# msi-se/generalized-icp

Hardware: AMD Instinct MI355X
Metric: GICP iterations/sec (and ms/iter) at N points, 1/2/4/8 GPU; final transform error (higher is better)
Workload: dtype f32-screen+f64; 1 GPU; 3d_room_1000k_1000k_k20; n_target=1000000, dim=3, k=20, parallelism=dp1 (one GPU, no collective)

## Files before the change

### generalized-icp_amd/csrc/gicp_kernels.hip

```cpp
#include <hip/hip_runtime.h>

#include <algorithm>
#include <utility>

#include "gicp_internal.h"
#include "gicp_solver.h"
#include "gicp_solve_dev.h"

namespace gicp {

__device__ __forceinline__ int lane_id() { return __lane_id(); }
__device__ __forceinline__ unsigned umed3(unsigned a, unsigned b, unsigned c) {
    return max(min(a, b), min(max(a, b), c));
}
__device__ __forceinline__ float key_d2(unsigned k) { return __uint_as_float(k & ~63u); }
__device__ __forceinline__ float marg(const Margin& m, float d2) {
    return fmaf(m.a * 1.0001f, __builtin_amdgcn_sqrtf(d2), fmaf(m.c, d2, m.b));
}

#define GICP_WAVE_REDUCE(OP, ID, x)                                                      \
    x = OP(x, __builtin_amdgcn_update_dpp(ID, x, 0x111, 0xf, 0xf, false));               \
    x = OP(x, __builtin_amdgcn_update_dpp(ID, x, 0x112, 0xf, 0xf, false));               \
    x = OP(x, __builtin_amdgcn_update_dpp(ID, x, 0x114, 0xf, 0xf, false));               \
    x = OP(x, __builtin_amdgcn_update_dpp(ID, x, 0x118, 0xf, 0xf, false));               \
// ... 312 lines not shown
        qa.ew[a] = 0.5f * (hi - lo) + 4.8e-7f * (fabsf(lo) + fabsf(hi) + B) + 1e-30f;
    }
    return qa;
}

struct NoCount {
    __device__ __forceinline__ void count(int, unsigned = 1) {}
};
template <int D, class Visit, class WB, class Collect, class Cnt = NoCount>
__device__ __forceinline__ void traverse_c(const DevCloud& db, const Query<D>& q, int seed, Visit&& visit,
                                           WB&& wave_bound, float skin, Collect&& collect, Cnt* cnt = nullptr) {
    const int l = lane_id();
    auto infl = [&](float w) -> float {
        if (skin <= 0.f || w < 0.f) return w;
        const float r = __builtin_amdgcn_sqrtf(w) * 1.0001f + skin;
        return r * r;
    };
    float wb = wave_bound();
    float wbi = infl(wb);
    if (seed >= 0) {
        collect(seed);
        if (visit(seed)) {
            wb = wave_bound();
            wbi = infl(wb);
        }
    }
    typedef __attribute__((address_space(4))) const BlockInfo* ConstBlocks;
    const ConstBlocks cb0 = (ConstBlocks)(uintptr_t)db.blocks + db.nblocks;
    for (int b0 = 0; b0 < db.nblocks; b0 += kWave) {
        {
            const ConstBlocks sb = cb0 + (b0 / kWave);
            const double c[3] = {sb->c[0], sb->c[1], sb->c[2]};
            const float h[3] = {sb->h[0], sb->h[1], sb->h[2]};
            if (!__builtin_amdgcn_readfirstlane((int)(gap2_box<D>(q, c, h) <= wbi))) continue;
        }
        if (cnt) cnt->count(5);
        const int b = b0 + l;
        bool cb = false;
        if (b < db.nblocks) cb = gap2_box<D>(q, db.blocks[b].c, db.blocks[b].h) <= wbi;
        uint64_t bm = __ballot(cb);
        while (bm) {
            const int bb = b0 + __ffsll((unsigned long long)bm) - 1;
            bm &= bm - 1;
            const int first = db.blocks[bb].first, nt = db.blocks[bb].ntiles;
            if (cnt) cnt->count(6);
            const int t = first + l;
            bool ct = false, cv = false;
            if (l < nt && t != seed) {
                const float g2 = gap2_box<D>(q, db.tiles[t].c, db.tiles[t].h);
                ct = g2 <= wbi;
                cv = g2 <= wb;
            }
            if (skin > 0.f) {
                uint64_t cm = __ballot(ct);
                while (cm) {
                    collect(first + __ffsll((unsigned long long)cm) - 1);
                    cm &= cm - 1;
                }
            }
            uint64_t tm = __ballot(cv);
            while (tm) {
                const int T = first + __ffsll((unsigned long long)tm) - 1;
                tm &= tm - 1;
                if (visit(T)) {
                    wb = wave_bound();
                    wbi = infl(wb);
                }
            }
        }
    }
}

template <int D, class Visit, class WB>
__device__ __forceinline__ void traverse(const DevCloud& db, const Query<D>& q, int seed, Visit&& visit,
                                         WB&& wave_bound) {
    traverse_c<D>(db, q, seed, visit, wave_bound, 0.f, [](int) {});
}

struct WaveStage {
    float x[kTile], y[kTile], z[kTile];
    double x64[kTile], y64[kTile], z64[kTile];
    int32_t perm[kTile];
};
constexpr int kStatRow = 17;
constexpr int kStatU = 12, kStatV = 10;
struct WaveStat {
    double u[kStatU * kStatRow];
    double v[kStatV * kStatRow];
};
union __attribute__((aligned(16))) WaveLds {
    WaveStage t;
    WaveStat st;
};

template <int D>
__device__ __forceinline__ float lane_gap2(const Query<D>& q, const TileInfo& ti, float* pr) {
    float g2 = 0.f;
#pragma unroll
    for (int a = 0; a < D; ++a) {
        pr[a] = q.pw[a] + (float)(q.ow[a] - ti.c[a]);
        const float ap = fabsf(pr[a]);
        float g = ap - ti.h[a] - (ap + ti.h[a]) * 9.5367431640625e-7f;
        g = fmaxf(g, 0.f);
        g2 = fmaf(g, g, g2);
    }
    return g2;
}

typedef __attribute__((address_space(4))) const TileInfo* ConstTiles;
__device__ __forceinline__ TileInfo tile_meta(const DevCloud& db, int T) {
    const ConstTiles ct = (ConstTiles)(uintptr_t)db.tiles + __builtin_amdgcn_readfirstlane(T);
    TileInfo t;
#pragma unroll
    for (int a = 0; a < 3; ++a) {
        t.c[a] = ct->c[a];
        t.h[a] = ct->h[a];
    }
    t.start = ct->start;
    t.count = ct->count;
    t.radius = ct->radius;
#pragma unroll
    for (int g = 0; g < kSub; ++g)
#pragma unroll
        for (int a = 0; a < 3; ++a) {
            t.sc[a][g] = ct->sc[a][g];
            t.sh[a][g] = ct->sh[a][g];
        }
    return t;
}

__device__ __forceinline__ void stage_f32(const DevCloud& db, const TileInfo& ti, WaveLds& L) {
    const int l = lane_id();
    float4 v = make_float4(1e30f, 1e30f, 1e30f, 0.f);
    if (l < ti.count) v = db.rel32[ti.start + l];
    L.t.x[l] = v.x;
    L.t.y[l] = v.y;
    L.t.z[l] = v.z;
    wave_sync();
}
__device__ __forceinline__ float4 load_rel(const DevCloud& db, int start, int count) {
    const int l = lane_id();
    float4 v = make_float4(1e30f, 1e30f, 1e30f, 0.f);
    if (l < count) v = db.rel32[start + l];
    return v;
}
__device__ __forceinline__ void stage_f32_from(const float4& v, WaveLds& L) {
    const int l = lane_id();
    L.t.x[l] = v.x;
    L.t.y[l] = v.y;
    L.t.z[l] = v.z;
    wave_sync();
}
template <int D, class VisitPre, class WB, class Collect, class Cnt = NoCount>
__device__ __forceinline__ void walk_c(const DevCloud& db, const Query<D>& q, int seed, VisitPre&& visit_pre,
                                       WB&& wave_bound, float skin, Collect&& collect, Cnt* cnt = nullptr) {
    const int l = lane_id();
    auto infl = [&](float w) -> float {
        if (skin <= 0.f || w < 0.f) return w;
        const float r = __builtin_amdgcn_sqrtf(w) * 1.0001f + skin;
        return r * r;
    };
    float wb = wave_bound();
    float wbi = infl(wb);
    if (seed >= 0) {
        collect(seed);
        if (visit_pre(seed, nullptr)) {
            wb = wave_bound();
// ... 494 lines not shown
            return wave_maxf(amb ? b64 + 2.f * marg(A.mg, b64) : -1.f);
        });
    }

    if (q.valid) {
        A.cov_out[i] = cov_descriptor<D>(S, A.min_nb, A.eps_a, A.m_scale);
        A.count_out[i] = (int)S.n;
    }
}

__global__ void __launch_bounds__(256) k_graph_pack(const float4* __restrict__ nb, const float2* __restrict__ nbh,
                                                    int64_t n, uint4* __restrict__ nbq, uint4* __restrict__ nbx,
                                                    int32_t* __restrict__ nbi) {
    const int64_t i = (int64_t)blockIdx.x * blockDim.x + threadIdx.x;
    if (i >= n) return;
    const float2 h = nbh[i];
    const int cnt = __float_as_int(h.y);
    float m = 0.f;
    for (int k = 0; k < cnt; ++k) {
        const float4 v = nb[i * kGraphK + k];
        m = fmaxf(m, fmaxf(fabsf(v.x), fmaxf(fabsf(v.y), fabsf(v.z))));
    }
    const float s = m > 0.f ? m / 32767.f : 1e-30f;
    const float inv = 1.f / s;
    float key[kGraphK];
    int ord[kGraphK];
    for (int k = 0; k < cnt; ++k) {
        const float4 v = nb[i * kGraphK + k];
        const float kk = fmaf(v.z, v.z, fmaf(v.y, v.y, v.x * v.x));
        const int t = __float_as_int(v.w);
        int pos = k;
        while (pos > 0 && (key[pos - 1] > kk || (key[pos - 1] == kk && __float_as_int(nb[i * kGraphK + ord[pos - 1]].w) > t))) {
            key[pos] = key[pos - 1];
            ord[pos] = ord[pos - 1];
            --pos;
        }
        key[pos] = kk;
        ord[pos] = k;
    }
    uint32_t w[2 + 2 * kGraphK];
    w[0] = __float_as_uint(h.x);
    w[1] = __float_as_uint(s);
    int q[4] = {0, 0, 0, 0};
    for (int k = 0; k < kGraphK; ++k) {
        int idx = -1;
        if (k < cnt) {
            const float4 v = nb[i * kGraphK + ord[k]];
            const float c[3] = {v.x, v.y, v.z};
            for (int a = 0; a < 3; ++a) q[a] = max(-32767, min(32767, __float2int_rn(c[a] * inv)));
            idx = __float_as_int(v.w);
            const int64_t d = (int64_t)idx - i;
            q[3] = d >= -32767 && d <= 32767 ? (int)d : kGraphFar;
        }
        w[2 + 2 * k] = ((uint32_t)q[0] & 0xFFFFu) | ((uint32_t)q[1] << 16);
        w[3 + 2 * k] = ((uint32_t)q[2] & 0xFFFFu) | ((uint32_t)q[3] << 16);
        nbi[i * kGraphK + k] = idx;
    }
    for (int c = 0; c < 8; ++c) nbq[i * 8 + c] = make_uint4(w[4 * c], w[4 * c + 1], w[4 * c + 2], w[4 * c + 3]);
    uint32_t x[12] = {};
    for (int k = 0; k < 2 * (kGraphK - kGraphLineA); ++k) x[k] = w[2 + 2 * kGraphLineA + k];
    for (int c = 0; c < 3; ++c) nbx[i * 3 + c] = make_uint4(x[4 * c], x[4 * c + 1], x[4 * c + 2], x[4 * c + 3]);
}

#ifndef GICP_CORR_ATTR
#if defined(GICP_CORR_WAVES_PER_EU)
#define GICP_CORR_ATTR __attribute__((amdgpu_num_sgpr(GICP_CORR_SGPR), amdgpu_waves_per_eu(GICP_CORR_WAVES_PER_EU, GICP_CORR_WAVES_PER_EU)))
#else
#define GICP_CORR_ATTR __attribute__((amdgpu_num_sgpr(GICP_CORR_SGPR), amdgpu_waves_per_eu(6, 6)))
#endif
#endif
#ifndef GICP_CORR_SGPR
#define GICP_CORR_SGPR 100
#endif

template <int D>
struct StatIdx {
    static constexpr int NS = D * (D + 1) / 2;
    static constexpr int pa(int p) { return D == 3 ? (p < 3 ? 0 : (p < 5 ? 1 : 2)) : (p < 2 ? 0 : 1); }
    static constexpr int pb(int p) {
        return D == 3 ? (p == 0 ? 0 : p == 1 ? 1 : p == 2 ? 2 : p == 3 ? 1 : 2) : (p == 0 ? 0 : 1);
    }
};

template <int D>
__device__ __forceinline__ double stat_value(int k, const double (&W)[D][D], const double (&s)[D],
                                             const double (&wr)[D], double rwr) {
    using SI = StatIdx<D>;
    constexpr int NS = SI::NS;
    if (k < NS * NS) {
        const int p = k / NS, qd = k % NS;
        return W[SI::pa(p)][SI::pb(p)] * (s[SI::pa(qd)] * s[SI::pb(qd)]);
    }
    k -= NS * NS;
    if (k < NS * D) return W[SI::pa(k / D)][SI::pb(k / D)] * s[k % D];
    k -= NS * D;
    if (k < NS) return W[SI::pa(k)][SI::pb(k)];
    k -= NS;
    if (k < D * D) return wr[k / D] * s[k % D];
    k -= D * D;
    if (k < D) return wr[k];
    k -= D;
    if (k == 0) return rwr;
    return 1.0;
}

#ifndef GICP_SPARSE_GROUP
#define GICP_SPARSE_GROUP 4
#endif
constexpr int kSparseGroup = GICP_SPARSE_GROUP;

template <int NV>
__device__ bool peer_exchange(const PeerArgs P, uint64_t seq, double* vals) {
    static_assert(NV <= kPeerSlot, "an exchange slot holds the values");
    __shared__ int s_fail;
    const int R = P.n, me = P.rank, tid = (int)threadIdx.x, nt = (int)blockDim.x;
    const int par = (int)(seq & 1u);
    for (int p = 0; p < R; ++p) {
        double* const dst = P.area[p] + kPeerFlagWords + (size_t)(par * kMaxPeers + me) * kPeerSlot;
        for (int k = tid; k < NV; k += nt) __hip_atomic_store(dst + k, vals[k], __ATOMIC_RELAXED, __HIP_MEMORY_SCOPE_SYSTEM);
    }
    __threadfence_system();
    if (tid == 0) s_fail = 0;
    __syncthreads();
    if (tid < R) {
        uint64_t* f = reinterpret_cast<uint64_t*>(P.area[tid]) + par * kMaxPeers + me;
        __hip_atomic_store(f, seq, __ATOMIC_RELEASE, __HIP_MEMORY_SCOPE_SYSTEM);
        if (tid == 0) *P.ctr = seq;
        const uint64_t* g = reinterpret_cast<const uint64_t*>(P.own) + par * kMaxPeers + tid;
        const uint64_t t0 = (uint64_t)wall_clock64();
        while (__hip_atomic_load(g, __ATOMIC_ACQUIRE, __HIP_MEMORY_SCOPE_SYSTEM) != seq) {
            if ((uint64_t)wall_clock64() - t0 > P.timeout) {
                s_fail = 1;
                break;
            }
            __builtin_amdgcn_s_sleep(1);
        }
    }
    __syncthreads();
    if (s_fail) return false;
    __builtin_amdgcn_fence(__ATOMIC_ACQUIRE, "");
    for (int k = tid; k < NV; k += nt) {
        double s = 0.0;
        for (int p = 0; p < R; ++p)
            s += __hip_atomic_load(P.own + kPeerFlagWords + (size_t)(par * kMaxPeers + p) * kPeerSlot + k,
                                   __ATOMIC_RELAXED, __HIP_MEMORY_SCOPE_SYSTEM);
        vals[k] = s;
    }
    __syncthreads();
    return true;
}

__device__ __forceinline__ double probe_value(int rank, int k, int r) {
    return ldexp((double)((rank + 1) * 1000003 + k * 97 + r * 7919), -7);
}
__global__ void __launch_bounds__(64) k_peer_probe(PeerArgs P, int rounds, double* out) {
    __shared__ double v[kPeerSlot];
    __shared__ uint64_t s_seq;
    __shared__ int s_bad;
    if (threadIdx.x == 0) {
        s_seq = *P.ctr;
        s_bad = 0;
    }
    int done = 0;
    for (int r = 0; r < rounds; ++r) {
        for (int k = threadIdx.x; k < kPeerSlot; k += blockDim.x) v[k] = probe_value(P.rank, k, r);
        __syncthreads();
// ... 52 lines not shown
        const void* p0 = A.state;
        const void* p1 = sc.tiles;
        const void* p2 = A.cert_pass;
        const void* p3 = A.hint;
        asm volatile("" ::"s"(p0), "s"(p1), "s"(p2), "s"(p3));
    }
    const ConstState cs0 = (ConstState)(uintptr_t)A.state;
    const TileInfo st = tile_meta(sc, Tq);
    const int cpass0 = ((ConstI32)(uintptr_t)A.cert_pass)[Tq];
    const int hint0 = ((ConstI32)(uintptr_t)A.hint)[Tq];
    const bool done = cs0->converged && !A.single_pass;
    struct {
        double R[9], t[3];
        float R32[9];
    } P;
#pragma unroll
    for (int a = 0; a < D; ++a) {
#pragma unroll
        for (int b = 0; b < D; ++b) {
            P.R[a * D + b] = cs0->T[a * (D + 1) + b];
            P.R32[a * D + b] = (float)P.R[a * D + b];
        }
        P.t[a] = cs0->T[a * (D + 1) + D];
    }

#ifdef GICP_TAIL
    unsigned long long tl[kTailWords] = {};
    __shared__ unsigned s_walk[8];
    if (threadIdx.x < 8) s_walk[threadIdx.x] = 0;
    __syncthreads();
    if (A.tail && blockIdx.x == 0 && threadIdx.x == 0) A.tail[0] = __builtin_amdgcn_s_memrealtime();
#define GICP_TAIL_MARK(k) do { if (A.tail) tl[k] = __builtin_amdgcn_s_memrealtime(); } while (0)
#else
#define GICP_TAIL_MARK(k) do {} while (0)
#endif
    Stamps S;
    S.start();
#ifdef GICP_TIMELINE
    if (A.stamps && l == 0)
        A.stamps[((int64_t)blockIdx.x * kCorrWaves + w) * 20 + 16] = __builtin_amdgcn_s_memrealtime();
    S.ta = tl_after(P.R[0] + st.c[0], cpass0 + hint0 + st.count);
#endif
    if ((A.use_lists || A.cert_j) && blockIdx.x == 0 && threadIdx.x == 0 && !done) {
        double* ring = A.poses + (A.pass % kPoseRing) * 12;
        for (int a = 0; a < 3; ++a) {
            for (int b = 0; b < 3; ++b) ring[a * 3 + b] = (a < D && b < D) ? P.R[a * D + b] : 0.0;
            ring[9 + a] = a < D ? P.t[a] : 0.0;
        }
    }
    int pairs = 0, list_rebuilds = 0, namb_total = 0, ngproved = 0, nwalked = 0;
    if (T < 0 && done) return;
    if (T >= 0) {
    bool on = false;
    double W[D][D] = {}, sv[D] = {}, wr[D] = {}, rwr = 0.0, r2 = 0.0;
    bool amb = false;
    {
        if (done) return;
        Query<D> q;
        q.valid = l < st.count;
        int i = st.start + min(l, st.count - 1);
        auto refresh_i = [&]() {
            i = st.start + min(lane_id(), st.count - 1);
            asm volatile("" : "+v"(i));
        };
        const float4 rel = sc.rel32[i];
        const float relv[3] = {rel.x, rel.y, rel.z};
#pragma unroll
        for (int a = 0; a < D; ++a) {
            double o = P.t[a];
            float pw = 0.f, ew = 0.f;
#pragma unroll
            for (int b = 0; b < D; ++b) {
                o += P.R[a * D + b] * st.c[b];
                pw = fmaf(P.R32[a * D + b], relv[b], pw);
                ew = fmaf(fabsf(P.R32[a * D + b]), st.h[b], ew);
            }
            q.ow[a] = o;
            q.pw[a] = pw;
            q.ew[a] = ew * (1.0f + 4.8e-7f) + 1e-30f;
        }
        const bool lists = A.use_lists != 0;

        int seed = hint0;
        if (seed < 0 || seed >= tg.ntiles) {
            const uint32_t code = morton_code(q.ow, D, tg.lo, tg.scale, tg.bits);
            int lo = 0, hi = tg.ntiles - 1;
            if (tg.seed_tab) {
                const uint32_t b = code >> tg.seed_shift;
                lo = tg.seed_tab[b];
                hi = tg.seed_tab[b + 1];
            }
            while (lo < hi) {
                const int mid = (lo + hi + 1) >> 1;
                if (tg.tile_code[mid] <= code) lo = mid;
                else hi = mid - 1;
            }
            seed = lo;
        }

        auto disp_since = [&](int bp) -> float {
            if (bp < 0 || A.pass - bp <= 0 || A.pass - bp >= kPoseRing) return -1.f;
            const double* Pb = A.poses + (bp % kPoseRing) * 12;
            double dc2 = 0.0, dr2 = 0.0;
#pragma unroll
            for (int a = 0; a < D; ++a) {
                double m = P.t[a] - Pb[9 + a];
#pragma unroll
                for (int b = 0; b < D; ++b) {
                    const double dr = P.R[a * D + b] - Pb[a * 3 + b];
                    m += dr * st.c[b];
                    dr2 += dr * dr;
                }
                dc2 += m * m;
            }
            return (__builtin_amdgcn_sqrtf((float)dc2) + __builtin_amdgcn_sqrtf((float)dr2) * st.radius) * 1.0001f + 1e-30f;
        };

        bool cert = false;
        int cj = -1;
        float cgap = 0.f, cdelta = -1.f;
        int jp = -1;
        if (A.cert_j) {
            jp = A.cert_j[i];
            const float g0 = A.cert_gap[i];
            cdelta = disp_since(cpass0);
            if constexpr (D == 3) cdelta = __int_as_float(__builtin_amdgcn_readfirstlane(__float_as_int(cdelta)));
            if (cdelta >= 0.f && q.valid) {
                cj = jp;
                cgap = g0;
                cert = cj >= 0 ? 2.f * cdelta < cgap : cgap - cdelta > A.empty_r;
            }
        }
#ifdef GICP_TIMELINE
        S.tb = tl_after(rel.x + cgap, jp);
#endif
        bool have_jp = false;
        float qr[3] = {0.f, 0.f, 0.f}, d2jp = 0.f;
        uint32_t w0[16];
        if (A.cert_j && q.valid && !cert && jp >= 0 && jp < tg.n) {
            const double4 t4 = reinterpret_cast<const double4*>(tg.xyz64)[jp];
            if (tg.nbq) {
                const uint4* row = tg.nbq + (int64_t)jp * 8;
#pragma unroll
                for (int c = 0; c < 4; ++c) {
                    const uint4 v = row[c];
                    w0[4 * c] = v.x;
                    w0[4 * c + 1] = v.y;
                    w0[4 * c + 2] = v.z;
                    w0[4 * c + 3] = v.w;
                }
            }
            const double tv[3] = {t4.x, t4.y, t4.z};
#pragma unroll
            for (int a = 0; a < D; ++a) {
                qr[a] = (float)(q.ow[a] - tv[a]) + q.pw[a];
                d2jp = fmaf(qr[a], qr[a], d2jp);
            }
            have_jp = true;
        }
        bool gcert = false;
        float ggap = 0.f;
#ifdef GICP_TAIL
        int gwhy = 0;
        int gout = 0;
#define GICP_WHY(k) (gwhy = (k))
#define GICP_OUT(k) (gout = (k))
#else
// ... 74 lines not shown
                        coords(k + 1, cb);
                        const f2v ms = {-sc, -sc};
                        const f2v dx = __builtin_elementwise_fma(ms, f2v{ca[0], cb[0]}, f2v{qr[0], qr[0]});
                        const f2v dy = __builtin_elementwise_fma(ms, f2v{ca[1], cb[1]}, f2v{qr[1], qr[1]});
                        const f2v dz = __builtin_elementwise_fma(ms, f2v{ca[2], cb[2]}, f2v{qr[2], qr[2]});
                        const f2v dd = __builtin_elementwise_fma(dx, dx, __builtin_elementwise_fma(dy, dy, dz * dz));
                        upd(dd.x, k);
                        upd(dd.y, k + 1);
                    };
                    auto entries = [&](int k0, int k1) {
#pragma unroll
                        for (int k = k0; k + 1 < k1; k += 2) entry2(k);
                        if ((k1 - k0) & 1) entry(k1 - 1);
                    };
                    auto reach = [&](int k) -> float {
                        float c[3];
                        coords(k, c);
                        const float ox = sc * c[0], oy = sc * c[1], oz = sc * c[2];
                        return __builtin_amdgcn_sqrtf(fmaf(ox, ox, fmaf(oy, oy, oz * oz)));
                    };
                    entries(0, kGraphHalf);
                    const float d0 = __builtin_amdgcn_sqrtf(d0s);
                    const float e = eq + 0.87f * sc + kGraphErr * (d0 + r);
                    float lc = reach(kGraphHalf - 1) - sc - d0 - 2.f * e;
                    bool need = lc <= __builtin_amdgcn_sqrtf(b1) + 2.f * e;
                    if (wave_any(need)) {
                        if (need) {
                            load_half(4);
                            entries(kGraphHalf, kGraphLineA);
                            lc = reach(kGraphLineA - 1) - sc - d0 - 2.f * e;
                            need = lc <= __builtin_amdgcn_sqrtf(b1) + 2.f * e;
                        }
                        if (wave_any(need)) {
                            if (need) {
                                const uint4* rx = tg.nbx + (int64_t)node * 3;
#pragma unroll
                                for (int c = 0; c < 2; ++c) {
                                    const uint4 v = rx[c];
                                    xb[4 * c] = v.x;
                                    xb[4 * c + 1] = v.y;
                                    xb[4 * c + 2] = v.z;
                                    xb[4 * c + 3] = v.w;
                                }
                                const uint2 v2 = *reinterpret_cast<const uint2*>(rx + 2);
                                xb[8] = v2.x;
                                xb[9] = v2.y;
                                entries(kGraphLineA, kGraphK);
                            }
                        }
                    }
                    if (!need) b2 = fminf(b2, lc * lc);
                    auto next_index = [&]() -> int {
                        const int bd = (int)wb >> 16;
                        return bd != kGraphFar ? node + bd : tg.nbi[(int64_t)node * kGraphK + bk];
                    };
                    const float e1 = __builtin_amdgcn_sqrtf(b1), e2 = __builtin_amdgcn_sqrtf(b2);
                    if (e2 - e1 <= 2.f * e) {
                        tie = d0 + e1 + 2.f * e < r;
                        tfar = r - d0 - e;
                        tnode = node;
                        act = false;
                        if (!tie) GICP_WHY(2);
                    } else if (d0 + e1 + 2.f * e < r) {
                        gcert = true;
                        GICP_OUT(h > 0 ? 3 : bk < 0 ? 1 : 2);
                        cj = bk < 0 ? node : next_index();
                        ggap = fminf(e2, r - d0) - e1 - 2.f * e;
                        act = false;
                    } else if (bk < 0) {
                        act = false;
                        GICP_WHY(1);
                    } else {
                        const float c0 = (float)(((int)(wa << 16)) >> 16), c1 = (float)((int)wa >> 16);
                        const float c2 = (float)(((int)(wb << 16)) >> 16);
                        qr[0] = fmaf(-sc, c0, qr[0]);
                        qr[1] = fmaf(-sc, c1, qr[1]);
                        qr[2] = fmaf(-sc, c2, qr[2]);
                        eq = e;
                        node = next_index();
                    }
                }
            }
            if (act) GICP_WHY(3);
            if (wave_any(tie)) {
                if (tie) {
                    double p64[D];
                    {
                        const double4 s4 = reinterpret_cast<const double4*>(A.src.xyz64)[i];
                        const double s4v[3] = {s4.x, s4.y, s4.z};
#pragma unroll
                        for (int a = 0; a < D; ++a) {
                            double p = P.t[a];
#pragma unroll
                            for (int b = 0; b < D; ++b) p += P.R[a * D + b] * s4v[b];
                            p64[a] = p;
                        }
                    }
                    double bd2 = 1e300, sd2 = 1e300;
                    int bj = -1, bo = 0x7fffffff;
                    auto consider = [&](int t) {
                        const double4 t4 = reinterpret_cast<const double4*>(tg.xyz64)[t];
                        const double tv[3] = {t4.x, t4.y, t4.z};
                        const double d2 = dist2_exact<D>(tv, p64);
                        const int og = tg.perm[t];
                        if (d2 < bd2 || (d2 == bd2 && og < bo)) {
                            sd2 = bd2;
                            bd2 = d2;
                            bj = t;
                            bo = og;
                        } else {
                            sd2 = fmin(sd2, d2);
                        }
                    };
                    consider(tnode);
                    const int32_t* ri = tg.nbi + (int64_t)tnode * kGraphK;
                    for (int k = 0; k < kGraphK; ++k) {
                        const int t = ri[k];
                        if (t >= 0) consider(t);
                    }
                    gcert = bj >= 0;
                    if (gcert) GICP_OUT(4);
                    cj = bj;
                    const double g = (fmin(sqrt(sd2), (double)tfar) - sqrt(bd2)) * (1.0 - 1e-6) - 1e-12;
                    ggap = g > 0.0 ? (float)g * (1.0f - 1e-6f) : 0.f;
                }
            }
            if (gcert) {
                cert = true;
                cgap = ggap;
            }
        }
        const bool any_gcert = wave_any(gcert);
        const bool skip_walk = !wave_any(q.valid && !cert);
#ifdef GICP_TAIL
        if (A.tail) {
            const bool wl = q.valid && !cert;
            const uint64_t wm = __ballot(wl);
            const int cd = __popcll(__ballot(have_jp));
            if (l == 0 && cd) atomicAdd(&s_walk[0], (unsigned)cd);
            for (int k = 1; k <= 4; ++k) {
                const int c = __popcll(__ballot(gout == k));
                if (l == 0 && c) atomicAdd(&s_walk[k], (unsigned)c);
            }
            if (l == 0 && wm) {
                atomicAdd(&s_walk[5], (unsigned)__popcll(wm));
                atomicAdd(&s_walk[6], 1u);
            }
            (void)gwhy;
        }
#endif
        ngproved = __popcll(__ballot(gcert));
        nwalked = skip_walk ? 0 : 1;
#ifdef GICP_TIMELINE
        S.tdesc = tl_after(ngproved, (int)skip_walk);
        S.ndesc = (unsigned)__popcll(__ballot(have_jp));
        S.nwalk = (unsigned)__popcll(__ballot(q.valid && !cert));
        S.nwalk_jp = (unsigned)__popcll(__ballot(q.valid && !cert && have_jp));
#endif
        const float kap = cdelta > A.kappa ? 0.f : A.kappa;

        const unsigned init = __float_as_uint(A.search2) | 63u;
        unsigned best = init, sec = init;
        int best_tile = -1;
        auto bound_of = [&](float b) -> float {
            const float w = b + 2.f * marg(A.mg, b);
            const float r = __builtin_amdgcn_sqrtf(b) + kap;
            return fmaxf(w, r * r);
        };
        float cap = 3e38f;
        if (have_jp && !cert && !skip_walk) cap = bound_of(d2jp + 2.f * marg(A.mg, d2jp)) * 1.0001f;
        auto lane_bound = [&]() -> float {
            if (!q.valid || cert) return -1.f;
            return fminf(cap, fminf(key_d2(sec), bound_of(key_d2(best))));
        };
        float lb = lane_bound();
#ifdef GICP_TIMELINE
        S.wb0 = __builtin_amdgcn_sqrtf(fmaxf(wave_maxf(lb), 0.f));
#endif
        auto inflate = [&](float w) -> float {
            if (w < 0.f) return w;
            const float r = __builtin_amdgcn_sqrtf(w) * 1.0001f + 2.f * A.gap_slack;
            return r * r;
        };
        float lbx = inflate(lb);
        int lvis = -1;
        auto visit_pre = [&](int Tt, const float4* pre) -> bool {
            if (wave_any(lvis == Tt)) return false;
            S.mark(1);
            S.count(0);
            const TileInfo ti = tile_meta(tg, Tt);
            float pr[D];
            if (!wave_any(lane_gap2_ns<D>(q, ti, pr) <= lbx)) {
                S.mark(2);
                return false;
            }
            const unsigned sub = sub_mask_ns<D>(ti, pr, lbx);
            if (pre) stage_f32_from(*pre, L);
            else stage_f32(tg, ti, L);
            S.mark(2);
            unsigned tb = 0xFFFFFFFFu, ts = 0xFFFFFFFFu;
            scan_tile<D>(L, ti.count, pr, [&](unsigned key, int) {
                ts = umed3(tb, ts, key);
                tb = min(tb, key);
            }, sub);
            pairs += rows_scanned(sub, ti.count);
            S.count(1);
            S.count(2, __popc(sub));
            if (tb < best) {
                sec = min(best, ts);
                best = tb;
                best_tile = Tt;
            } else {
                sec = min(sec, tb);
            }
            lb = lane_bound();
            lbx = inflate(lb);
            wave_sync();
            S.mark(3);
            return true;
        };
        S.mark(0);
        bool use = false;
        float delta = 0.f, rc = 0.f;
        int nl = 0;
        if (lists && !skip_walk) {
            nl = A.list_len[T];
            rc = A.list_rcert[T];
            if (nl > 0 && rc > 0.f) {
                delta = disp_since(A.list_pass[T]);
                use = delta >= 0.f && delta < rc;
            }
        }
        int ent = 0;

        const uint64_t walkers = skip_walk ? 0ull : __ballot(lb >= 0.f);
        const bool sparse = walkers != 0ull && __popcll(walkers) <= A.sparse_max;
        auto sparse_search = [&](int wl) {
            float pw[D];
#pragma unroll
            for (int a = 0; a < D; ++a) pw[a] = readlane_f(q.pw[a], wl);
            Query<D> qp = q;
#pragma unroll
            for (int a = 0; a < D; ++a) {
                const float B = 2.f * q.ew[a] + 1e-30f;
                qp.ow[a] = q.ow[a] + (double)pw[a];
                qp.ew[a] = 4.8e-7f * (2.f * fabsf(pw[a]) + B) + 1e-30f;
            }
            const float capw = readlane_f(cap, wl);
            float wb = readlane_f(lb, wl);
            unsigned tb = init, ts = init;
            int tt = -1;
            unsigned wbest = init, wsec = init;
            int wtile = -1;
            const unsigned M = key_mask();
            auto reduce = [&]() {
                wbest = wave_min_key(tb);
                const int win = __ffsll((unsigned long long)__ballot(tb == wbest)) - 1;
                wsec = wave_min_key(l == win ? ts : tb);
                wtile = __builtin_amdgcn_readlane(tt, win);
                wb = fminf(capw, fminf(key_d2(wsec), bound_of(key_d2(wbest))));
            };
            auto screen = [&](uint64_t cm, int ct, int cst, int ccnt, const float* co, float cg) {
                cm &= __ballot(cg <= wb);
                while (cm) {
                    int ks[kSparseGroup];
                    float rx[kSparseGroup], ry[kSparseGroup], rz[kSparseGroup];
#pragma unroll
// ... 170 lines not shown
            };
            walk_c<D>(tg, q, seed, visit_pre, [&]() { return wave_maxf(lb); }, lists ? skin : 0.f,
                      collect, &S);
            if (lists) {
                const float wbf = wave_maxf(lb);
                const float r = ncol <= kListMax ? __builtin_amdgcn_sqrtf(fmaxf(wbf, 0.f)) * 0.9999f + skin : 0.f;
                if (ncol <= kListMax) {
                    float key = 3e38f;
                    if (l < ncol) {
                        key = 0.f;
#pragma unroll
                        for (int a = 0; a < D; ++a) {
                            const float d = (float)(tg.boxes[cent].c[a] - q.ow[a]);
                            key = fmaf(d, d, key);
                        }
                    }
                    wave_sort64(key, cent);
                    if (l < ncol) A.list[(int64_t)T * kListMax + l] = cent;
                }
                if (l == 0) {
                    A.list_len[T] = min(ncol, kListMax);
                    A.list_rcert[T] = r;
                    A.list_pass[T] = A.pass;
                }
            }
        }
        S.mark(1);
#ifdef GICP_TIMELINE
        S.twalk = tl_after(best, best_tile);
        S.kind = skip_walk ? 0u : use_sparse ? 4u : use ? 1u : list_rebuilds > 0 ? 2u : 3u;
#endif

        auto source_point = [&](const double4& s4) {
            const double s4v[3] = {s4.x, s4.y, s4.z};
#pragma unroll
            for (int a = 0; a < D; ++a) {
                double p = P.t[a];
#pragma unroll
                for (int b = 0; b < D; ++b) p += P.R[a * D + b] * s4v[b];
                q.p64[a] = p;
            }
        };
        refresh_i();
        if (!skip_walk) source_point(reinterpret_cast<const double4*>(sc.xyz64)[i]);
        const bool found = cert ? cj >= 0 : (q.valid && best < init);
        int j = -1;
        double d2e = 0.0;
        if (cert) {
            j = cj;
        } else if (found) {
            const float b = key_d2(best), s2 = key_d2(sec);
            amb = (s2 - b) <= marg(A.mg, b) + marg(A.mg, s2);
            j = tg.boxes[best_tile].start + (int)(best & 63u);
        }
        if (A.cert_j && (!skip_walk || any_gcert || A.pass - cpass0 >= kPoseRing / 2)) {
            if (q.valid) {
                float g = 0.f;
                if (gcert) {
                    g = cgap;
                } else if (cert) {
                    g = cj >= 0 ? cgap - 2.f * cdelta : cgap - cdelta;
                } else if (found) {
                    if (!amb) {
                        const float b = key_d2(best), s2 = key_d2(sec);
                        const float lo2 = fminf(s2 - marg(A.mg, s2), lane_bound());
                        const float hi2 = b + marg(A.mg, b);
                        g = (__builtin_amdgcn_sqrtf(fmaxf(lo2, 0.f)) - __builtin_amdgcn_sqrtf(hi2)) * 0.999f;
                    }
                } else {
                    g = __builtin_amdgcn_sqrtf(A.search2 - marg(A.mg, A.search2)) * 0.9999f;
                }
                A.cert_j[i] = cert ? cj : (found && !amb ? j : -1);
                A.cert_gap[i] = (found && amb) ? 0.f : g;
            }
            if (l == 0) A.cert_pass[T] = A.pass;
        }
        const uint64_t fm = __ballot(found && !cert);
        if (fm && A.hint) {
            const int src_lane = __ffsll((unsigned long long)fm) - 1;
            const int bt = __shfl(best_tile, src_lane);
            if (l == 0) A.hint[T] = bt;
        }

        if (!skip_walk && __any(amb)) {
            double bd2 = 1e300;
            float sd2 = 3e38f;
            int bj = -1;
            const float lim = key_d2(best) + 2.f * marg(A.mg, key_d2(best));
            auto visit64 = [&](int Tt) -> bool {
                const TileInfo ti = tile_meta(tg, Tt);
                float pr[D];
                const bool need = amb && lane_gap2<D>(q, ti, pr) <= lim;
                if (!__any(need)) return false;
                S.count(7);
                const unsigned sub = sub_mask<D>(ti, pr, amb, lim);
                stage_f64(tg, ti, L);
                if (l < ti.count) L.t.perm[l] = tg.perm[ti.start + l];
                wave_sync();
                for (int g = 0; g < kSub; ++g) {
                    if (!((sub >> g) & 1u)) continue;
                    const int je = min(kSubRows * g + kSubRows, ti.count);
#pragma unroll 4
                    for (int jj = kSubRows * g; jj < je; ++jj) {
                        const double qq[3] = {L.t.x64[jj], L.t.y64[jj], L.t.z64[jj]};
                        const double d2 = dist2_exact<D>(qq, q.p64);
                        const int og = L.t.perm[jj];
                        if (amb) {
                            if (d2 < bd2 || (d2 == bd2 && bj >= 0 && og < tg.perm[bj])) {
                                sd2 = (float)bd2 * 0.99999976f;
                                bd2 = d2;
                                bj = ti.start + jj;
                            } else {
                                sd2 = fminf(sd2, (float)d2 * 0.99999976f);
                            }
                        }
                    }
                }
                wave_sync();
                return true;
            };
            const uint64_t am = __ballot(amb);
            if (__popcll(am) <= A.sparse_amb) {
                uint64_t wm = am;
                while (wm) {
                    const int wl = __ffsll((unsigned long long)wm) - 1;
                    wm &= wm - 1;
                    double pa[3] = {0.0, 0.0, 0.0};
                    Query<D> qp = q;
#pragma unroll
                    for (int a = 0; a < D; ++a) {
                        pa[a] = readlane_d(q.p64[a], wl);
                        const float pw = readlane_f(q.pw[a], wl);
                        const float B = 2.f * q.ew[a] + 1e-30f;
                        qp.ow[a] = q.ow[a] + (double)pw;
                        qp.ew[a] = 4.8e-7f * (2.f * fabsf(pw) + B) + 1e-30f;
                    }
                    const float limw = readlane_f(lim, wl);
                    double ub = 1e300;
                    int uo = 0x7fffffff, uj = -1;
                    float us = 3e38f;
                    auto screen64 = [&](uint64_t cm, int ts, int tc) {
                        while (cm) {
                            const int k = __ffsll((unsigned long long)cm) - 1;
                            cm &= cm - 1;
                            const int s0 = __builtin_amdgcn_readlane(ts, k), c0 = __builtin_amdgcn_readlane(tc, k);
                            S.count(7);
                            double d2 = 1e300;
                            int og = 0x7fffffff;
                            if (l < c0) {
                                const double4 x = reinterpret_cast<const double4*>(tg.xyz64)[s0 + l];
                                og = tg.perm[s0 + l];
                                const double xv[3] = {x.x, x.y, x.z};
                                d2 = dist2_exact<D>(xv, pa);
                            }
                            const double m = wave_mind(d2);
                            const uint64_t eq = __ballot(d2 == m);
                            const int om = (int)wave_min_key(d2 == m ? (unsigned)og : 0x7fffffffu);
                            const int wn = __ffsll((unsigned long long)__ballot(d2 == m && og == om)) - 1;
                            const double st = __popcll(eq) >= 2 ? m : wave_mind(l == wn ? 1e300 : d2);
                            if (m < ub || (m == ub && om < uo)) {
                                us = fminf(us, fminf((float)ub * 0.99999976f, (float)st * 0.99999976f));
                                ub = m;
                                uo = om;
                                uj = s0 + wn;
                            } else {
                                us = fminf(us, (float)m * 0.99999976f);
                            }
                        }
                    };
                    const int nsuper = (tg.nblocks + kWave - 1) / kWave;
                    for (int s0 = 0; s0 < nsuper; s0 += kWave) {
                        float sg = 3e38f;
                        if (s0 + l < nsuper) sg = gap2_box<D>(qp, tg.blocks[tg.nblocks + s0 + l].c, tg.blocks[tg.nblocks + s0 + l].h);
                        uint64_t sm = __ballot(sg <= limw);
                        while (sm) {
                            const int sl = __ffsll((unsigned long long)sm) - 1;
                            sm &= sm - 1;
                            const int b0 = (s0 + sl) * kWave, b = b0 + l;
                            float bg = 3e38f;
                            if (b < tg.nblocks) bg = gap2_box<D>(qp, tg.blocks[b].c, tg.blocks[b].h);
                            uint64_t bm = __ballot(bg <= limw);
                            while (bm) {
                                const int bl = __ffsll((unsigned long long)bm) - 1;
                                bm &= bm - 1;
                                const int first = (b0 + bl) * kBlockTiles, nt = min(kBlockTiles, tg.ntiles - first);
// ... 91 lines not shown
                    W[0][1] = W[1][0] = -S[0][1] * id;
                } else {
                    const double c00 = S[1][1] * S[2][2] - S[1][2] * S[2][1];
                    const double c01 = S[0][2] * S[2][1] - S[0][1] * S[2][2];
                    const double c02 = S[0][1] * S[1][2] - S[0][2] * S[1][1];
                    const double c11 = S[0][0] * S[2][2] - S[0][2] * S[2][0];
                    const double c12 = S[0][2] * S[1][0] - S[0][0] * S[1][2];
                    const double c22 = S[0][0] * S[1][1] - S[0][1] * S[1][0];
                    const double det = S[0][0] * c00 + S[0][1] * c01 + S[0][2] * c02;
                    const double id = solver_detail::recip(det);
                    W[0][0] = c00 * id;
                    W[0][1] = W[1][0] = c01 * id;
                    W[0][2] = W[2][0] = c02 * id;
                    W[1][1] = c11 * id;
                    W[1][2] = W[2][1] = c12 * id;
                    W[2][2] = c22 * id;
                }
                }
                double r[D];
#pragma unroll
                for (int a = 0; a < D; ++a) r[a] = qv[a] - q.p64[a];
                r2 = 0.0;
#pragma unroll
                for (int a = 0; a < D; ++a) r2 += r[a] * r[a];
                rwr = 0.0;
#pragma unroll
                for (int a = 0; a < D; ++a) {
                    wr[a] = 0.0;
#pragma unroll
                    for (int b = 0; b < D; ++b) wr[a] += W[a][b] * r[b];
                    rwr += r[a] * wr[a];
                }
            }
            if (A.dbg_index) A.dbg_index[sc.perm[i]] = on ? (int64_t)tg.perm[j] : -1;
        } else if (q.valid) {
            if (skip_walk) source_point(s4e);
            if (A.dbg_index) A.dbg_index[sc.perm[i]] = -1;
            if (A.dbg_dist) A.dbg_dist[sc.perm[i]] = 1.0 / 0.0;
        }
        if (A.dbg_det && q.valid) {
            double dt = 0.0;
            if (on) {
                if constexpr (D == 2) dt = W[0][0] * W[1][1] - W[0][1] * W[1][0];
                else
                    dt = W[0][0] * (W[1][1] * W[2][2] - W[1][2] * W[2][1]) -
                         W[0][1] * (W[1][0] * W[2][2] - W[1][2] * W[2][0]) +
                         W[0][2] * (W[1][0] * W[2][1] - W[1][1] * W[2][0]);
            }
            A.dbg_det[i] = dt;
            A.top_tgt[i] = on ? (int64_t)tg.perm[j] : -1;
        }
        if (A.dbg_weight && q.valid) {
            double* o = A.dbg_weight + (int64_t)sc.perm[i] * D * D;
#pragma unroll
            for (int a = 0; a < D; ++a)
#pragma unroll
                for (int b = 0; b < D; ++b) o[a * D + b] = on ? W[a][b] : 0.0;
        }
        amb = amb && q.valid;
    }

    S.mark(5);
    {
        constexpr int NS = D * (D + 1) / 2;
        constexpr int NU = NS + D + 3;
        constexpr int NV = NS + D + 1;
        auto uel = [&](int k) -> double {
            if (k < NS) return W[StatIdx<D>::pa(k)][StatIdx<D>::pb(k)];
            if (k < NS + D) return wr[k - NS];
            if (k == NS + D) return rwr;
            if (k == NS + D + 1) return on ? 1.0 : 0.0;
            return r2;
        };
        auto vel = [&](int k) -> double {
            if (k < NS) return sv[StatIdx<D>::pa(k)] * sv[StatIdx<D>::pb(k)];
            if (k < NS + D) return sv[k - NS];
            return 1.0;
        };
        typedef double d4v __attribute__((ext_vector_type(4)));
        d4v acc = {0.0, 0.0, 0.0, 0.0};
        WaveStat& X = s_lds[w].st;
        static_assert(NU <= kStatU && NV <= kStatV, "statistics terms fit the transpose image");
        const uint64_t onm = __ballot(on);
        wave_sync();
        double* const wu = &X.u[l & 15];
        double* const wv = &X.v[l & 15];
        const double* const ru = &X.u[min(l & 15, NU - 1) * kStatRow + (l >> 4)];
        const double* const rv = &X.v[min(l & 15, NV - 1) * kStatRow + (l >> 4)];
#pragma unroll
        for (int g = 0; g < 4; ++g) {
            if (((onm >> (16 * g)) & 0xFFFFull) == 0) continue;
            if ((l >> 4) == g) {
#pragma unroll
                for (int k = 0; k < NU; ++k) wu[k * kStatRow] = uel(k);
#pragma unroll
                for (int k = 0; k < NV; ++k) wv[k * kStatRow] = vel(k);
            }
            wave_sync();
#pragma unroll
            for (int cc = 0; cc < 4; ++cc) {
                if (((onm >> (16 * g + 4 * cc)) & 0xFull) == 0) continue;
                acc = __builtin_amdgcn_mfma_f64_16x16x4f64(ru[4 * cc], rv[4 * cc], acc, 0, 0, 0);
            }
            wave_sync();
        }
        double* const wst = wstat(w);
        for (int k = l; k < NSX; k += 64) wst[k] = 0.0;
#pragma unroll
        for (int j = 0; j < 4; ++j) {
            const int p = (l >> 4) + 4 * j, qq = l & 15;
            int idx = -1;
            if (p < NS) {
                if (qq < NS) idx = p * NS + qq;
                else if (qq < NS + D) idx = NS * NS + p * D + (qq - NS);
                else if (qq == NS + D) idx = NS * NS + NS * D + p;
            } else if (p < NS + D) {
                if (qq >= NS && qq < NS + D) idx = NS * NS + NS * D + NS + (p - NS) * D + (qq - NS);
                else if (qq == NS + D) idx = NS * NS + NS * D + NS + D * D + (p - NS);
            } else if (qq == NS + D && p <= NS + D + 1) {
                idx = NS * NS + NS * D + NS + D * D + D + (p - NS - D);
            } else if (qq == NS + D && p == NS + D + 2) {
                idx = NSS + 3;
            }
            if (idx >= 0) wst[idx] = acc[j];
        }
        namb_total += (int)__popcll(__ballot(amb));
    }
    } else {
        for (int k = l; k < NSX; k += 64) wstat(w)[k] = 0.0;
    }
    if (l == 0) {
        double* const wst = wstat(w);
        wst[NSS] = (double)namb_total;
        wst[NSS + 1] = (double)pairs * 64.0;
        wst[NSS + 2] = (double)list_rebuilds;
        wst[NSS + 4] = (double)ngproved;
        wst[NSS + 5] = (double)nwalked;
    }
    S.mark(6);
#if defined(GICP_STAMPS) || defined(GICP_TIMELINE)
#ifndef GICP_TIMELINE
    S.acc[7] = (unsigned long long)pairs;
#endif
    if (A.stamps && l == 0) {
        unsigned long long* o = A.stamps + ((int64_t)blockIdx.x * kCorrWaves + w) * 20;
#ifndef GICP_TIMELINE
        for (int c = 0; c < 8; ++c) o[c] = S.acc[c];
        for (int c = 0; c < 8; ++c) o[8 + c] = S.cnt[c];
#endif
#ifndef GICP_TIMELINE
        o[16] = S.rt0;
#else
        o[0] = (unsigned)T;
        o[1] = __float_as_uint(st.radius);
        o[2] = (unsigned)st.count;
        o[3] = S.tdesc;
        o[4] = S.twalk;
        o[5] = S.kind | (S.ndesc << 8) | (S.nwalk << 16) | (S.nwalk_jp << 24);
        o[6] = S.ta;
        o[7] = S.tb;
        for (int c = 0; c < 8; ++c) o[8 + c] = S.cnt[c];
        o[10] = S.te;
        o[12] = tl_after(pairs, namb_total);
        o[14] = __float_as_uint(S.wb0);
#endif
        o[17] = __builtin_amdgcn_s_memrealtime();
        o[18] = (unsigned)__builtin_amdgcn_s_getreg((31 << 11) | 4);
        o[19] = (unsigned)__builtin_amdgcn_s_getreg((31 << 11) | 20);
    }
#endif
    __syncthreads();
    __shared__ int s_last;
    for (int t = threadIdx.x; t < NSX; t += 64 * kCorrWaves) {
        double s = 0.0;
#pragma unroll
        for (int u = 0; u < kCorrWaves; ++u) s += wstat(u)[t];
        __hip_atomic_store(&A.partials[(int64_t)unit * NSX + t], s, __ATOMIC_RELAXED, __HIP_MEMORY_SCOPE_AGENT);
    }
    asm volatile("s_waitcnt vmcnt(0)" ::: "memory");
    GICP_TAIL_MARK(1);
#ifdef GICP_TAIL
    if (A.tail && threadIdx.x < 7 && s_walk[threadIdx.x]) atomicAdd(A.tail + 9 + threadIdx.x, (unsigned long long)s_walk[threadIdx.x]);
#endif
    __syncthreads();
    const bool flat = nunits <= kFlatUnits;
    const int ng = flat ? 1 : (nunits + kGroupWG - 1) / kGroupWG;
    const int g = flat ? 0 : unit / kGroupWG;
    if (threadIdx.x == 0) {
        const int gn = flat ? nunits : min(kGroupWG, nunits - g * kGroupWG);
        uint32_t* const tk = flat ? &A.tickets[kMaxGroups * kTicketStride] : &A.tickets[g * kTicketStride];
        s_last = __hip_atomic_fetch_add(tk, 1u, __ATOMIC_RELAXED, __HIP_MEMORY_SCOPE_AGENT) == (unsigned)(gn - 1);
        if (s_last) {
            __builtin_amdgcn_fence(__ATOMIC_ACQUIRE, "agent");
            asm volatile("s_waitcnt vmcnt(0)" ::: "memory");
        }
        GICP_TAIL_MARK(2);
    }
    __syncthreads();
    if (!s_last) return;
    static_assert(sizeof(double) * 4 * NSX <= sizeof(WaveLds) * kCorrWaves, "reduction scratch fits the staging LDS");
    double (*s_red)[NSX] = reinterpret_cast<double (*)[NSX]>(&s_lds[0]);
    double* s_sum = reinterpret_cast<double*>(&s_lds[0]) + 3 * NSX;
    auto sum_rows = [&](const double* src, int b0, int b1, double* dst_stat) {
        constexpr int PART = 27;
        constexpr int NP = (64 * kCorrWaves) / NSX >= 3 ? 3 : 1;
        constexpr int NT = 64 * kCorrWaves;
        const int tid = threadIdx.x;
// ... 404 lines not shown
```

Before: 21890 it/s.

## Halve MFMA stat-reduction passes and table-drive stat slot indices

The per-wave statistics transpose now stages 32 lanes per pass (row stride 33), so two LDS fill/sync rounds replace four, and it issues eight unconditional f64 MFMAs per round. The per-lane index arithmetic that maps accumulator entries to statistic slots is replaced by a constexpr byte-packed lookup table held in device memory. Branch hints mark the seed search, tie resolution and ambiguous-point paths as unlikely, the lane bound is skipped when no walk happens, and the exact fallback loops are no longer unrolled. In exchange, LDS use for the stat image roughly doubles, MFMAs now run even for inactive lane groups, and each lane adds a global table load.

Result: faster. 23760 it/s, median of 6 (+8.5%).

```diff
diff --git a/generalized-icp_amd/csrc/gicp_kernels.hip b/generalized-icp_amd/csrc/gicp_kernels.hip
--- a/generalized-icp_amd/csrc/gicp_kernels.hip
+++ b/generalized-icp_amd/csrc/gicp_kernels.hip
@@ -418,7 +418,7 @@
     double x64[kTile], y64[kTile], z64[kTile];
     int32_t perm[kTile];
 };
-constexpr int kStatRow = 17;
+constexpr int kStatRow = 33;
 constexpr int kStatU = 12, kStatV = 10;
 struct WaveStat {
     double u[kStatU * kStatRow];
@@ -1079,6 +1079,55 @@
     }
 };
 
+constexpr int kNoSlot = 0xFF;
+template <int D>
+constexpr int stat_slot(int p, int q) {
+    constexpr int NS = D * (D + 1) / 2;
+    constexpr int oB = NS * NS, oC = oB + NS * D, oR = oC + NS, oT = oR + D * D, o0 = oT + D;
+    if (p < NS) {
+        if (q < NS) return p * NS + q;
+        if (q < NS + D) return oB + p * D + (q - NS);
+        if (q == NS + D) return oC + p;
+    } else if (p < NS + D) {
+        if (q >= NS && q < NS + D) return oR + (p - NS) * D + (q - NS);
+        if (q == NS + D) return oT + (p - NS);
+    } else if (q == NS + D) {
+        if (p <= NS + D + 1) return o0 + (p - NS - D);
+        if (p == NS + D + 2) return nstat(D) + 3;
+    }
+    return kNoSlot;
+}
+template <int D>
+struct StatSlots {
+    uint32_t lane[64];
+    constexpr StatSlots() : lane{} {
+        for (int l = 0; l < 64; ++l) {
+            uint32_t w = 0;
+            for (int j = 0; j < 4; ++j) w |= (uint32_t)stat_slot<D>((l >> 4) + 4 * j, l & 15) << (8 * j);
+            lane[l] = w;
+        }
+    }
+};
+static_assert(nstat_ext(3) <= kNoSlot && nstat_ext(2) <= kNoSlot, "a statistic's slot fits a byte");
+template <int D>
+constexpr bool stat_slots_one_owner() {
+    int owners[kNoSlot] = {};
+    for (int p = 0; p < 16; ++p)
+        for (int q = 0; q < 16; ++q)
+            if (stat_slot<D>(p, q) != kNoSlot) ++owners[stat_slot<D>(p, q)];
+    for (int k = 0; k < kNoSlot; ++k)
+        if (owners[k] != ((k < nstat(D) || k == nstat(D) + 3) ? 1 : 0)) return false;
+    return true;
+}
+static_assert(stat_slots_one_owner<2>() && stat_slots_one_owner<3>(), "one owner lane per statistic");
+__device__ const StatSlots<2> kStatSlots2{};
+__device__ const StatSlots<3> kStatSlots3{};
+template <int D>
+__device__ __forceinline__ uint32_t stat_slots(int l) {
+    if constexpr (D == 2) return kStatSlots2.lane[l];
+    else return kStatSlots3.lane[l];
+}
+
 template <int D>
 __device__ __forceinline__ double stat_value(int k, const double (&W)[D][D], const double (&s)[D],
                                              const double (&wr)[D], double rwr) {
@@ -1297,7 +1346,7 @@
         const bool lists = A.use_lists != 0;
 
         int seed = hint0;
-        if (seed < 0 || seed >= tg.ntiles) {
+        if (__builtin_expect(seed < 0 || seed >= tg.ntiles, 0)) {
             const uint32_t code = morton_code(q.ow, D, tg.lo, tg.scale, tg.bits);
             int lo = 0, hi = tg.ntiles - 1;
             if (tg.seed_tab) {
@@ -1538,7 +1587,7 @@
                 }
             }
             if (act) GICP_WHY(3);
-            if (wave_any(tie)) {
+            if (__builtin_expect(wave_any(tie), 0)) {
                 if (tie) {
                     double p64[D];
                     {
@@ -1629,7 +1678,8 @@
             if (!q.valid || cert) return -1.f;
             return fminf(cap, fminf(key_d2(sec), bound_of(key_d2(best))));
         };
-        float lb = lane_bound();
+        float lb = -1.f;
+        if (!skip_walk) lb = lane_bound();
 #ifdef GICP_TIMELINE
         S.wb0 = __builtin_amdgcn_sqrtf(fmaxf(wave_maxf(lb), 0.f));
 #endif
@@ -1638,7 +1688,8 @@
             const float r = __builtin_amdgcn_sqrtf(w) * 1.0001f + 2.f * A.gap_slack;
             return r * r;
         };
-        float lbx = inflate(lb);
+        float lbx = -1.f;
+        if (!skip_walk) lbx = inflate(lb);
         int lvis = -1;
         auto visit_pre = [&](int Tt, const float4* pre) -> bool {
             if (wave_any(lvis == Tt)) return false;
@@ -1975,7 +2026,7 @@
             if (l == 0) A.hint[T] = bt;
         }
 
-        if (!skip_walk && __any(amb)) {
+        if (__builtin_expect(!skip_walk && __any(amb), 0)) {
             double bd2 = 1e300;
             float sd2 = 3e38f;
             int bj = -1;
@@ -1990,10 +2041,11 @@
                 stage_f64(tg, ti, L);
                 if (l < ti.count) L.t.perm[l] = tg.perm[ti.start + l];
                 wave_sync();
+#pragma unroll 1
                 for (int g = 0; g < kSub; ++g) {
                     if (!((sub >> g) & 1u)) continue;
                     const int je = min(kSubRows * g + kSubRows, ti.count);
-#pragma unroll 4
+#pragma unroll 1
                     for (int jj = kSubRows * g; jj < je; ++jj) {
                         const double qq[3] = {L.t.x64[jj], L.t.y64[jj], L.t.z64[jj]};
                         const double d2 = dist2_exact<D>(qq, q.p64);
@@ -2251,15 +2303,16 @@
         WaveStat& X = s_lds[w].st;
         static_assert(NU <= kStatU && NV <= kStatV, "statistics terms fit the transpose image");
         const uint64_t onm = __ballot(on);
+        const uint32_t slots = stat_slots<D>(l);
         wave_sync();
-        double* const wu = &X.u[l & 15];
-        double* const wv = &X.v[l & 15];
+        double* const wu = &X.u[l & 31];
+        double* const wv = &X.v[l & 31];
         const double* const ru = &X.u[min(l & 15, NU - 1) * kStatRow + (l >> 4)];
         const double* const rv = &X.v[min(l & 15, NV - 1) * kStatRow + (l >> 4)];
 #pragma unroll
-        for (int g = 0; g < 4; ++g) {
-            if (((onm >> (16 * g)) & 0xFFFFull) == 0) continue;
-            if ((l >> 4) == g) {
+        for (int h = 0; h < 2; ++h) {
+            if ((uint32_t)(onm >> (32 * h)) == 0u) continue;
+            if ((l >> 5) == h) {
 #pragma unroll
                 for (int k = 0; k < NU; ++k) wu[k * kStatRow] = uel(k);
 #pragma unroll
@@ -2267,31 +2320,16 @@
             }
             wave_sync();
 #pragma unroll
-            for (int cc = 0; cc < 4; ++cc) {
-                if (((onm >> (16 * g + 4 * cc)) & 0xFull) == 0) continue;
+            for (int cc = 0; cc < 8; ++cc)
                 acc = __builtin_amdgcn_mfma_f64_16x16x4f64(ru[4 * cc], rv[4 * cc], acc, 0, 0, 0);
-            }
             wave_sync();
         }
         double* const wst = wstat(w);
         for (int k = l; k < NSX; k += 64) wst[k] = 0.0;
 #pragma unroll
         for (int j = 0; j < 4; ++j) {
-            const int p = (l >> 4) + 4 * j, qq = l & 15;
-            int idx = -1;
-            if (p < NS) {
-                if (qq < NS) idx = p * NS + qq;
-                else if (qq < NS + D) idx = NS * NS + p * D + (qq - NS);
-                else if (qq == NS + D) idx = NS * NS + NS * D + p;
-            } else if (p < NS + D) {
-                if (qq >= NS && qq < NS + D) idx = NS * NS + NS * D + NS + (p - NS) * D + (qq - NS);
-                else if (qq == NS + D) idx = NS * NS + NS * D + NS + D * D + (p - NS);
-            } else if (qq == NS + D && p <= NS + D + 1) {
-                idx = NS * NS + NS * D + NS + D * D + D + (p - NS - D);
-            } else if (qq == NS + D && p == NS + D + 2) {
-                idx = NSS + 3;
-            }
-            if (idx >= 0) wst[idx] = acc[j];
+            const int idx = (int)((slots >> (8 * j)) & 0xFFu);
+            if (idx != kNoSlot) wst[idx] = acc[j];
         }
         namb_total += (int)__popcll(__ballot(amb));
     }
```
